# mmwillet/TTS.cpp

Hardware: AMD Instinct MI355X
Metric: audio-seconds/sec (Parler-TTS-Mini fp16, greedy decode + DAC to 44.1 kHz PCM) (higher is better)
Workload: dtype f16

## Files before the change

### tts.cpp_amd/csrc/dac_b3_kernels.h

```cpp
#pragma once
#include <hip/hip_runtime.h>
#include <stdint.h>
#include <type_traits>

struct ResUnitGeom { int C, KS, KS2, WST, n7, ns1, n1; };
__host__ __device__ inline ResUnitGeom resunit_geom(int C, int KS, int KS2) {
    ResUnitGeom g;
    g.C = C; g.KS = KS; g.KS2 = KS2;
    const int a = 3 * KS * 2 * C * 8, b = 3 * KS2 * 2 * 96 * 8;
    g.WST = a > b ? a : b;
    g.n7 = (C / 8) * (4 / KS);
    g.ns1 = (C / 16) / KS2;
    g.n1 = (C / 96) * g.ns1;
    return g;
}

static __global__ void pack_resunit_b3_kernel(const float *w7, const float *w1, __bf16 *dst, int C, int KS, int KS2) {
    const ResUnitGeom g = resunit_geom(C, KS, KS2);
    const int64_t per7 = (int64_t) KS * 2 * C * 8, per1 = (int64_t) KS2 * 2 * 96 * 8;
    const int64_t total = (int64_t) g.n7 * per7 + (int64_t) g.n1 * per1;
    for (int64_t i = (int64_t) blockIdx.x * blockDim.x + threadIdx.x; i < total; i += (int64_t) gridDim.x * blockDim.x) {
        float v = 0.0f;
        int64_t base, plane_sz;
        if (i < (int64_t) g.n7 * per7) {
// ... 30 lines not shown
        dst[base + 2 * plane_sz] = h3;
    }
}

template <int N, typename F>
__device__ __forceinline__ void static_for(F &&f) {
    if constexpr (N > 0) {
        static_for<N - 1>(f);
        f(std::integral_constant<int, N - 1>{});
    }
}

struct ResUnitArgs {
    const float *x;
    float *y;
    const __bf16 *w;
    const float *b7, *b1;
    const float *alpha_in;
    const float *alpha_mid;
    int L, dil, pad;
    const uint32_t *frames;
    int mult;
    long long *stamps;
};
#define RU_STAMP(k) do { if (a.stamps && tid == 0) a.stamps[((int64_t) blockIdx.z * gridDim.x + blockIdx.x) * 5 + (k)] = (long long) __builtin_readcyclecounter(); } while (0)

template <int MI, int KS, int KS2, int SCHED = 1, int ABL = 0>
__global__ __launch_bounds__(512, 2) void resunit_b3_kernel(ResUnitArgs a) {
    constexpr int C = 32 * MI, WN = 8, NT = 512, T_T = 32 * WN;
    constexpr int SPC = 4 / KS;
    constexpr int WPL7 = KS * 2 * C * 8, WPL1 = KS2 * 2 * 96 * 8;
    constexpr int WST = 3 * (WPL7 > WPL1 ? WPL7 : WPL1);
    constexpr int NCH = C / 8, N7 = NCH * SPC, NP = MI / 3, NS1 = (C / 16) / KS2, N1 = NP * NS1;
    constexpr int WV = (WST / 8 + NT - 1) / NT;
    static_assert(4 % KS == 0 && (C / 16) % KS2 == 0 && MI % 3 == 0, "stage shapes");
    extern __shared__ __attribute__((aligned(16))) char smem[];
    const int xw = T_T + 6 * a.dil;
    const int xpl = xw * 8;
    __bf16 *wsb = (__bf16 *) smem;
    __bf16 *xsb = wsb + 2 * WST;
    float4 *tab = (float4 *) (xsb + 2 * 3 * xpl);
    float2 *tin = (float2 *) (tab + C);
    const int tid = threadIdx.x, lane = tid & 63, wn = tid >> 6;
    const int l31 = lane & 31, hi = lane >> 5;
    const int t0 = blockIdx.x * T_T;
    const int LS = a.L, L = valid_len(a.frames, a.mult, a.L);
// ... 499 lines not shown
        }
}

static __global__ void pack_convt_w_b3_kernel(const float *src, __bf16 *dst, int cout, int cin, int S, int CO_T, int n_chunks, int scheme = 0) {
    const int64_t plane_sz = (int64_t) 2 * S * 2 * CO_T * 8;
    const int64_t total = (int64_t) ((cout + CO_T - 1) / CO_T) * n_chunks * plane_sz;
    for (int64_t i = (int64_t) blockIdx.x * blockDim.x + threadIdx.x; i < total; i += (int64_t) gridDim.x * blockDim.x) {
        const int j = (int) (i % 8);
        int64_t r = i / 8;
        const int col = (int) (r % CO_T); r /= CO_T;
        const int hi = (int) (r % 2); r /= 2;
        const int ph = (int) (r % S); r /= S;
        const int ks = (int) (r % 2); r /= 2;
        const int ch = (int) (r % n_chunks);
        const int ct = (int) (r / n_chunks);
        const int co = ct * CO_T + col, ci = ch * 16 + ks * 8 + j, k = ph + hi * S;
        float v = 0.0f;
        if (co < cout && ci < cin) v = src[((int64_t) ci * cout + co) * 2 * S + k];
        const int64_t base = ((int64_t) ct * n_chunks + ch) * split_planes(scheme) * plane_sz + (i % plane_sz);
        split_store(scheme, v, dst, base, plane_sz);
    }
}

template <int S, int MI, bool PLANES = false, typename SP = SplitB3>
__global__ __launch_bounds__(512, 2) void convt_b3_kernel(ConvTArgs a) {
    constexpr int NPL = SP::NPL;
    constexpr int CO_T = 32 * MI, WN = 8, TI_T = 32 * WN, NT = 64 * WN, K2 = 2 * S;
    constexpr int WPL = 2 * S * 2 * CO_T * 8;
    constexpr int WV = (NPL * WPL / 8 + NT - 1) / NT;
    constexpr int xw = TI_T + 1;
    constexpr int XR = (2 * xw + NT - 1) / NT;
    constexpr int xpl = 2 * xw * 8;
    extern __shared__ __attribute__((aligned(16))) char smem[];
    __bf16 *wsb = (__bf16 *) smem;
    __bf16 *xsb = wsb + 2 * NPL * WPL;
    float2 *tin = (float2 *) (xsb + 2 * NPL * xpl);
    const int tid = threadIdx.x, lane = tid & 63, wn = tid >> 6;
    const int l31 = lane & 31, hi = lane >> 5;
    const TileId tile = xcd_tile(a.npos, a.nco, a.nz);
    if (!tile.valid) return;
    const int ti0 = tile.pos * TI_T, co0 = tile.co * CO_T;
    const int n_chunks = a.cin / 16;
    const int LS = a.L, L = valid_len_z(a.frames, a.mult, a.L, tile.z);
    const int LoS = a.Lout, Lout = a.frames ? (L - 1) * S - 2 * a.pad + K2 : a.Lout;
    if (ti0 > L) return;
    const float *xg = a.x + (int64_t) tile.z * a.cin * LS;
    const int64_t psti = (int64_t) (a.cin / 8) * LS * 8;
    const __bf16 *xpg = PLANES ? a.xp + (int64_t) tile.z * NPL * psti : nullptr;
    float *yg = a.y + (int64_t) tile.z * a.cout * LoS;
    const uint4d *wg = (const uint4d *) ((const __bf16 *) a.w + (int64_t) tile.co * n_chunks * NPL * WPL);

    if (!PLANES) {
        for (int i = tid; i < a.cin; i += NT) {
            const float al = a.alpha ? a.alpha[i] : 1.0f;
            tin[i] = make_float2(al, 1.0f / al);
        }
    }

    float16d acc[MI][S];
#pragma unroll
    for (int i = 0; i < MI; i++)
#pragma unroll
        for (int ph = 0; ph < S; ph++)
#pragma unroll
            for (int e = 0; e < 16; e++) acc[i][ph][e] = 0.0f;

    uint4d wreg[WV];
    float xreg[PLANES ? 1 : XR][8];
    uint4d xpreg[PLANES ? XR : 1][NPL];
    auto prefetch = [&](int c) __attribute__((always_inline)) {
        const uint4d *wp = wg + (int64_t) c * (NPL * WPL / 8);
#pragma unroll
        for (int j = 0; j < WV; j++) {
            const int i = tid + j * NT;
            if (i < NPL * WPL / 8) wreg[j] = wp[i];
        }
#pragma unroll
        for (int q = 0; q < XR; q++) {
            const int u = tid + q * NT;
            const int g = u / xw, r = u - g * xw;
            const int ti = ti0 - 1 + r;
            const bool ok = g < 2 && ti >= 0 && ti < L;
            if constexpr (PLANES) {
                const uint4d zero = {0u, 0u, 0u, 0u};
#pragma unroll
                for (int pl = 0; pl < NPL; pl++)
                    xpreg[q][pl] = ok ? *(const uint4d *) (xpg + pl * psti + ((int64_t) (c * 2 + g) * LS + ti) * 8) : zero;
            } else {
#pragma unroll
                for (int e = 0; e < 8; e++) xreg[q][e] = ok ? xg[(int64_t) (c * 16 + g * 8 + e) * LS + ti] : 0.0f;
            }
        }
    };
    auto commit = [&](int c, int buf) __attribute__((always_inline)) {
        uint4d *wd = (uint4d *) (wsb + buf * NPL * WPL);
#pragma unroll
        for (int j = 0; j < WV; j++) {
            const int i = tid + j * NT;
            if (i < NPL * WPL / 8) wd[i] = wreg[j];
        }
        __bf16 *xd = xsb + buf * NPL * xpl;
#pragma unroll
        for (int q = 0; q < XR; q++) {
            const int u = tid + q * NT;
            const int g = u / xw, r = u - g * xw;
            if constexpr (PLANES) {
                if (g < 2) {
                    __bf16 *p = xd + (g * xw + r) * 8;
#pragma unroll
                    for (int pl = 0; pl < NPL; pl++) *(uint4d *) (p + pl * xpl) = xpreg[q][pl];
                }
            } else if (g < 2) {
                if (a.alpha) {
                    float al[8], ral[8];
#pragma unroll
                    for (int e = 0; e < 8; e++) { const float2 t2 = tin[c * 16 + g * 8 + e]; al[e] = t2.x; ral[e] = t2.y; }
                    snake_vec<8>(xreg[q], al, ral);
                }
                bf16x8d hp[NPL];
#pragma unroll
                for (int e = 0; e < 8; e++) {
                    __bf16 pv[NPL];
// ... 113 lines not shown
            if (s >= cnt) continue;
            v = w7[((int64_t) co * C + chunk * 16 + hi * 8 + j) * 7 + first + s];
            plane_sz = (int64_t) cnt * 2 * C * 8;
            base = (int64_t) st * WST + ((int64_t) (s * 2 + hi) * C + co) * 8 + j;
        } else {
            const int64_t i1 = i - (int64_t) n7 * slot7;
            const int st = (int) (i1 / per1);
            int64_t r = i1 % per1;
            const int m = (int) (r % 8); r /= 8;
            const int col = (int) (r % 96); r /= 96;
            const int hi = (int) (r % 2); r /= 2;
            const int s = (int) r;
            const int pass = st / ns1, q = st % ns1;
            const int ks = q * KS2 + s, ib = ks / 2, qq = ks % 2;
            const int ch = 32 * ib + 16 * qq + (m < 4 ? 4 * hi + m : 8 + 4 * hi + m - 4);
            v = w1[(int64_t) (96 * pass + col) * C + ch];
            plane_sz = per1;
            base = (int64_t) (n7 + st) * WST + (i1 % per1);
        }
        split_store(scheme, v, dst, base, plane_sz);
    }
}

__device__ __forceinline__ void dac_wait_vmcnt0() { asm volatile("s_waitcnt vmcnt(0)" ::: "memory"); }
template <int MI, int KS2, typename SP = SplitB3, bool WDMA = false, int VAR = 0, int NI = 1>
__global__ __launch_bounds__(512, 2) void resunit_t7_kernel(ResUnitArgs a) {
    constexpr int NPL = SP::NPL;
    using G = ResT7<MI>;
    constexpr int C = 32 * MI, WN = 8, NT = 512, T_T = 32 * WN * NI, NQ = NI + 1;
    constexpr int SPC = G::SPC, NCH = C / 16, N7 = NCH * SPC;
    constexpr int WPL1 = KS2 * 2 * 96 * 8;
    constexpr int WST = NPL * G::MAXCNT * 2 * C * 8;
    constexpr int NP = MI / 3, NS1 = (C / 16) / KS2, N1 = NP * NS1;
    constexpr int WV = (WST / 8 + NT - 1) / NT;
    static_assert(NPL * WPL1 <= WST && (C / 16) % KS2 == 0 && MI % 3 == 0, "stage shapes");
    static_assert(NI == 1 || ((VAR & 2) != 0 && NPL <= 2 && N1 % 2 == 0), "NI > 1: once-built operand, an even number of k = 1 stages");
    extern __shared__ __attribute__((aligned(16))) char smem[];
    const int xw = T_T + 6 * a.dil;
    const int xpl = 2 * xw * 8;
    __bf16 *wsb = (__bf16 *) smem;
    __bf16 *xsb = wsb + 2 * WST;
    float4 *tab = (float4 *) (xsb + 2 * NPL * xpl);
    float2 *tin = (float2 *) (tab + C);
    const int tid = threadIdx.x, lane = tid & 63, wn = tid >> 6;
    const int l31 = lane & 31, hi = lane >> 5;
    const int t0 = blockIdx.x * T_T;
    const int LS = a.L, L = valid_len(a.frames, a.mult, a.L);
    if (t0 >= L) return;
    const float *xg = a.x + (int64_t) blockIdx.z * C * LS;
    float *yg = a.y + (int64_t) blockIdx.z * C * LS;
    const uint4d *wg = (const uint4d *) a.w;

    for (int i = tid; i < C; i += NT) {
        const float am = a.alpha_mid[i], ai = a.alpha_in[i];
        tab[i] = make_float4(a.b7[i], am, 1.0f / am, a.b1[i]);
        tin[i] = make_float2(ai, 1.0f / ai);
    }

    float16d acc[NI][MI];
#pragma unroll
    for (int j = 0; j < NI; j++)
#pragma unroll
        for (int i = 0; i < MI; i++)
#pragma unroll
            for (int e = 0; e < 16; e++) acc[j][i][e] = 0.0f;

    constexpr int NPIECE = WST * 2 / 1024;
    static_assert(!WDMA || (WST * 2) % 1024 == 0, "stage = whole 1-KiB pieces");
    uint4d wreg[WDMA ? 1 : WV];
    float xreg[NQ][8];
    auto prefetch_w = [&](int g) __attribute__((always_inline)) {
        if constexpr (WDMA) {
            const char *wp = (const char *) a.w + (int64_t) g * (WST * 2) + lane * 16;
            char *wd = (char *) (wsb + (g & 1) * WST);
#pragma unroll
            for (int j = 0; j < (NPIECE + 7) / 8; j++) {
                const int pc = wn + 8 * j;
                if (NPIECE % 8 == 0 || pc < NPIECE)
                    __builtin_amdgcn_global_load_lds((const __attribute__((address_space(1))) void *) (wp + pc * 1024),
// ... 184 lines not shown
#pragma unroll
                for (int pl = 0; pl < NPL; pl++)
                    af[ii][pl] = *(const bf16x8d *) (ws + pl * WPL1 + (((s * 2 + hi) * 96) + ii * 32 + l31) * 8);
#pragma unroll
            for (int tm = 0; tm < SP::NT; tm++)
#pragma unroll
                for (int ii = 0; ii < 3; ii++)
                    acc2[ii] = SP::mfma(af[ii][SP::ta(tm)], bf[SP::tb(tm)], acc2[ii]);
        });
        if constexpr (g2 + 1 < N1 || jt + 1 < NI) {
            commit_w((N7 + g2 + 1) & 1);
            __syncthreads();
        }
        if constexpr (q == NS1 - 1) {
            if (t < L) {
#pragma unroll
                for (int i = 0; i < 3; i++) {
                    float rv[16];
#pragma unroll
                    for (int e = 0; e < 16; e++) {
                        const int co = 96 * p + 32 * i + (e & 3) + 8 * (e >> 2) + 4 * hi;
                        rv[e] = xg[(int64_t) co * LS + t];
                    }
#pragma unroll
                    for (int e = 0; e < 16; e++) {
                        const int co = 96 * p + 32 * i + (e & 3) + 8 * (e >> 2) + 4 * hi;
                        yg[(int64_t) co * LS + t] = (acc2[i][e] + tab[co].w) + rv[e];
                    }
                }
            }
        }
    });
    });
    RU_STAMP(4);
}
```

### tts.cpp_amd/csrc/dac_kernels.h

```cpp
#pragma once
#include <hip/hip_runtime.h>
#include <stdint.h>

typedef float float4d __attribute__((ext_vector_type(4)));

__device__ __forceinline__ float snake_sin_poly(float x) {
    const float q = rintf(x * 0.318309886183790671537767526745028724f);
    float r = fmaf(q, -3.140625f, x);
    r = fmaf(q, -0.0009670257568359375f, r);
    r = fmaf(q, -6.2771141529083251953e-07f, r);
    r = fmaf(q, -1.2154201256553420762e-10f, r);
    const float s = r * r;
    if (((int) q) & 1) r = -r;
    float u = 2.6083159809786593541503e-06f;
    u = fmaf(u, s, -0.0001981069071916863322258f);
    u = fmaf(u, s, 0.00833307858556509017944336f);
    u = fmaf(u, s, -0.166666597127914428710938f);
    return fmaf(s, u * r, r);
}
__device__ __forceinline__ float snake_sin(float x) {
    if (!(fabsf(x) < 125.0f)) return sinf(x);
    return snake_sin_poly(x);
}

__device__ __forceinline__ float snake_f(float x, float alpha, float ralpha) {
    const float s = snake_sin(x * alpha);
    return x + (s * s) * ralpha;
}
template <int N>
__device__ __forceinline__ void snake_vec(float (&v)[N], const float (&al)[N], const float (&ral)[N]) {
    float arg[N];
    bool big = false;
#pragma unroll
    for (int e = 0; e < N; e++) { arg[e] = v[e] * al[e]; big = big || !(fabsf(arg[e]) < 125.0f); }
    if (__builtin_amdgcn_ballot_w64(big) != 0) {
#pragma unroll
        for (int e = 0; e < N; e++) { const float s = snake_sin(arg[e]); v[e] = v[e] + (s * s) * ral[e]; }
    } else {
#pragma unroll
        for (int e = 0; e < N; e++) { const float s = snake_sin_poly(arg[e]); v[e] = v[e] + (s * s) * ral[e]; }
    }
}
__device__ __forceinline__ float snake_ch(float x, int cig, int cin, int cin_pad, const float *als, const float *alpha, int tab) {
    if (tab) return snake_f(x, als[cig], als[cin_pad + cig]);
    const float al = cig < cin ? alpha[cig] : 1.0f;
    return snake_f(x, al, 1.0f / al);
}

struct DacEmbedArgs {
    const uint32_t *frames;
    const uint32_t *codes;
    const float *codebook;
    const float *proj_w;
    const float *proj_b;
    int n_cb, cb_size, cb_dim, latent, T;
    int Tout;
    float *out;
    int x_f16;
};

static __global__ void dac_embed_kernel(DacEmbedArgs a) {
    const int t = blockIdx.x * blockDim.x + threadIdx.x;
    const int c = blockIdx.y, z = blockIdx.z;
// ... 1382 lines not shown
```

### tts.cpp_amd/csrc/shim_codec.hip

```cpp
#include "shim_internal.h"

#include "dac_kernels.h"
#include "dac_b3_kernels.h"
#include "kokoro_kernels.h"

static int dac_snapshot(tts_hip_ctx *c, int stage, const float *dev, size_t C, size_t L, size_t LS) {
    if (!c->debug) return 0;
    HIPCHK(hipStreamSynchronize(c->stream));
    std::vector<float> &v = c->dac_dbg[stage];
    v.resize(C * L);
    HIPCHK(hipMemcpy2DAsync(v.data(), L * 4, dev, LS * 4, L * 4, C, hipMemcpyDeviceToHost, c->stream));
    HIPCHK(hipStreamSynchronize(c->stream));
    return 0;
}

#define CI32_K1 16
#ifndef CI32_T
#define CI32_T 8
#endif
#ifndef CI32_K7
#define CI32_K7 4
#endif
static int conv_tile(int cout, int K, int *CO_T, int *CI_T) {
    if (K != 7 && K != 1) return -1;
// ... 327 lines not shown
        else if (K == 1) hipLaunchKernelGGL(conv1d_kernel<1>, grid, dim3(256), lds, c->stream, a);
        else return set_err("conv1d: kernel size %d unsupported", K);
        HIPCHK(hipGetLastError());
    }
    return prof_end(c);
}

template <int S, int MI, int WM, int WN, int CI_T>
static int launch_convt_mfma(tts_hip_ctx *c, const ConvTArgs &a_in, int nz) {
    constexpr int CO_T = 32 * MI * WM, TI_T = 32 * WN, WCH = CI_T * 2 * S * CO_T;
    const int cin_pad = (a_in.cin + CI_T - 1) / CI_T * CI_T;
    ConvTArgs a = a_in;
    const size_t lds = dac_lds_request(c, ((size_t) 2 * WCH + 2 * (size_t) ((CI_T * (TI_T + 1) + 3) & ~3)) * 4, (a.alpha ? 2 * (size_t) cin_pad : 0) * 4, &a.alpha_tab, true);
    static std::atomic<uint64_t> attr{0};
    if (attr_needed(attr, c->device)) {
        HIPCHK(hipFuncSetAttribute((const void *) convt1d_mfma_kernel<S, MI, WM, WN, CI_T>, hipFuncAttributeMaxDynamicSharedMemorySize, 160 * 1024));
    }
    const dim3 grid((a.L + 1 + TI_T - 1) / TI_T, (a.cout + CO_T - 1) / CO_T, nz);
    hipLaunchKernelGGL((convt1d_mfma_kernel<S, MI, WM, WN, CI_T>), grid, dim3(64 * WM * WN), lds, c->stream, a);
    HIPCHK(hipGetLastError());
    return 0;
}

template <int S, int MI, bool PL, typename SP>
static int launch_convt_b3_t(tts_hip_ctx *c, const ConvTArgs &a, int nz) {
    constexpr int CO_T = 32 * MI, WPL = 2 * S * 2 * CO_T * 8, xpl = 2 * 257 * 8;
    const size_t lds = (size_t) 2 * SP::NPL * WPL * 2 + (size_t) 2 * SP::NPL * xpl * 2 + (size_t) a.cin * 8;
    if (lds > 160 * 1024) return set_err("convt_b3: %d input channels need %zu bytes of LDS", a.cin, lds);
    static std::atomic<uint64_t> attr{0};
    if (attr_needed(attr, c->device)) {
        HIPCHK(hipFuncSetAttribute((const void *) convt_b3_kernel<S, MI, PL, SP>, hipFuncAttributeMaxDynamicSharedMemorySize, 160 * 1024));
    }
    ConvTArgs b = a;
    b.npos = (a.L + 1 + 255) / 256; b.nz = nz;
    b.nco = xcd_order(a.cout / CO_T, (double) a.cin * a.L * nz * 4, (double) a.cout * a.cin * 2 * S * 6);
    hipLaunchKernelGGL((convt_b3_kernel<S, MI, PL, SP>), dim3(xcd_grid(b.npos, a.cout / CO_T, b.nz)), dim3(512), lds, c->stream, b);
    HIPCHK(hipGetLastError());
    return 0;
}
template <int S, int MI, typename SP>
static int launch_convt_b3_s(tts_hip_ctx *c, const ConvTArgs &a, int nz) {
    return a.xp ? launch_convt_b3_t<S, MI, true, SP>(c, a, nz) : launch_convt_b3_t<S, MI, false, SP>(c, a, nz);
}
template <int S, int MI>
static int launch_convt_b3(tts_hip_ctx *c, const ConvTArgs &a, int nz) {
    const int sc = dac_scheme(c);
    return sc == 0 ? launch_convt_b3_s<S, MI, SplitB3>(c, a, nz) : sc == 1 ? launch_convt_b3_s<S, MI, SplitH2>(c, a, nz) : launch_convt_b3_s<S, MI, SplitH1>(c, a, nz);
}

static int launch_convt(tts_hip_ctx *c, ConvTArgs ta, size_t w_off, int nz) {
    const bool valu = (c->d.flags & TTS_HIP_FLAG_VALU_GEMM) != 0;
    const int s = ta.stride;
    auto pct = c->packed_ct.find(w_off);
    if (!valu && c->dac_convt_b3 && pct != c->packed_ct.end()) {
        ta.w = (const float *) pct->second;
        ta.x_f16 = 0;
        if (s == 8) return launch_convt_b3<8, 1>(c, ta, nz);
        if (s == 4) return launch_convt_b3<4, 2>(c, ta, nz);
        return launch_convt_b3<2, 3>(c, ta, nz);
    }
    int CO_T = 0;
    const int cfg = valu ? -1 : convt_tile(ta.cout, s, &CO_T);
    ta.x_f16 = c->dac_f16 ? 1 : 0;
    auto pk16 = c->packed16.find(w_off);
// ... 69 lines not shown
        else CHK((launch_conv_b3p_t<7, 2, 2, 1, 4, 4, 2>(c, a, bt.n)));
    } else if (cout % 256 == 0) {
        CHK((launch_conv_b3p_t<1, 4, 2, 2, 4, 1, 2>(c, a, bt.n)));
    } else {
        CHK((launch_conv_b3p_t<1, 2, 4, 2, 4, 1, 2>(c, a, bt.n)));
    }
    return prof_end(c);
}

template <int MI, int KS, int KS2>
static int launch_resunit_t(tts_hip_ctx *c, const ResUnitArgs &a, int nz) {
    constexpr int C = 32 * MI;
    const ResUnitGeom g = resunit_geom(C, KS, KS2);
    const int xw = 256 + 6 * a.dil;
    const size_t lds = (size_t) 2 * g.WST * 2 + (size_t) 6 * xw * 8 * 2 + (size_t) C * 24;
    static std::atomic<uint64_t> attr{0};
    if (attr_needed(attr, c->device)) {
        HIPCHK(hipFuncSetAttribute((const void *) resunit_b3_kernel<MI, KS, KS2>, hipFuncAttributeMaxDynamicSharedMemorySize, 160 * 1024));
    }
    hipLaunchKernelGGL((resunit_b3_kernel<MI, KS, KS2>), dim3((a.L + 255) / 256, 1, nz), dim3(512), lds, c->stream, a);
    HIPCHK(hipGetLastError());
    return 0;
}
template <int MI, int KS2, typename SP, bool WDMA, int VAR, int NI = 1>
static int launch_resunit_t7_s(tts_hip_ctx *c, const ResUnitArgs &a, int nz) {
    constexpr int C = 32 * MI, T_T = 256 * NI;
    const int xw = T_T + 6 * a.dil;
    const size_t WST = (size_t) SP::NPL * ResT7<MI>::MAXCNT * 2 * C * 8;
    const size_t lds = 2 * WST * 2 + (size_t) 2 * SP::NPL * 2 * xw * 8 * 2 + (size_t) C * 24;
    static std::atomic<uint64_t> attr{0};
    if (attr_needed(attr, c->device)) {
        HIPCHK(hipFuncSetAttribute((const void *) resunit_t7_kernel<MI, KS2, SP, WDMA, VAR, NI>, hipFuncAttributeMaxDynamicSharedMemorySize, 160 * 1024));
    }
    hipLaunchKernelGGL((resunit_t7_kernel<MI, KS2, SP, WDMA, VAR, NI>), dim3((a.L + T_T - 1) / T_T, 1, nz), dim3(512), lds, c->stream, a);
    HIPCHK(hipGetLastError());
    return 0;
}
template <int MI, int KS2>
static int launch_resunit_t7(tts_hip_ctx *c, const ResUnitArgs &a, int nz) {
    const int sc = dac_scheme(c);
    constexpr int NI = MI == 3 ? 2 : 1;
    if (c->dac_wdma)
        return sc == 0 ? launch_resunit_t7_s<MI, KS2, SplitB3, true, 0>(c, a, nz) : sc == 1 ? launch_resunit_t7_s<MI, KS2, SplitH2, true, 2, NI>(c, a, nz) : launch_resunit_t7_s<MI, KS2, SplitH1, true, 2, NI>(c, a, nz);
    return sc == 0 ? launch_resunit_t7_s<MI, KS2, SplitB3, false, 0>(c, a, nz) : sc == 1 ? launch_resunit_t7_s<MI, KS2, SplitH2, false, 0>(c, a, nz) : launch_resunit_t7_s<MI, KS2, SplitH1, false, 0>(c, a, nz);
}
static bool resunit_fused(const tts_hip_ctx *c, const DRes &r, int dil) {
    return c->dac_fuse && !(c->d.flags & TTS_HIP_FLAG_VALU_GEMM) && dil <= 9 && c->packed_ru.count(r.in_w);
}
static int launch_resunit(tts_hip_ctx *c, const DacBatch &bt, const DRes &r, int C, int LS, int dil, const float *x, float *y) {
    ResUnitArgs a{};
    a.x = x; a.y = y; a.w = c->packed_ru.at(r.in_w);
    a.b7 = (const float *) (c->arena + r.in_b); a.b1 = (const float *) (c->arena + r.out_b);
    a.alpha_in = (const float *) (c->arena + r.in_alpha); a.alpha_mid = (const float *) (c->arena + r.out_alpha);
    a.L = LS; a.dil = dil; a.pad = 3 * dil; a.frames = bt.frames; a.mult = bt.mult;
    const double Lv = bt.tot_frames * bt.mult;
    CHK(prof_begin(c, TTS_HIP_K_DAC_RESUNIT, (2.0 * C * Lv + 8.0 * C * C) * 4, 2.0 * C * (double) C * 8 * Lv));
    if (c->dac_tap7) {
        if (C == 96) CHK((launch_resunit_t7<3, 3>(c, a, bt.n)));
        else CHK((launch_resunit_t7<6, 4>(c, a, bt.n)));
    } else if (C == 96) CHK((launch_resunit_t<3, 4, 3>(c, a, bt.n)));
    else CHK((launch_resunit_t<6, 2, 4>(c, a, bt.n)));
    return prof_end(c);
}

static int dac_decode_batch_on(tts_hip_ctx *c, const uint32_t *codes, const uint32_t *frames, uint32_t n, float *pcm_out);
static int dac_decode_batch(tts_hip_ctx *c, const uint32_t *codes, const uint32_t *frames, uint32_t n, float *pcm_out) {
    if (!c || !c->finalized || !c->has_dac) return set_err("tts_hip_dac_decode: context has no finalized DAC");
    if (!frames || !codes || !pcm_out) return set_err("tts_hip_dac_decode: null argument");
    const uint32_t G = (uint32_t) std::max(1, c->dac_group);
    size_t code_off = 0, pcm_off = 0;
    for (uint32_t g0 = 0; g0 < n; g0 += G) {
        const uint32_t m = std::min(G, n - g0);
        size_t fr = 0;
        for (uint32_t i = 0; i < m; i++) fr += frames[g0 + i];
        int rc;
        {
            std::lock_guard<std::mutex> lock(g_dac_pass_mutex[(unsigned) c->device % 64]);
            if (!c->dac_stream) {
                rc = dac_decode_batch_on(c, codes + code_off * c->d_ncb, frames + g0, m, pcm_out + pcm_off);
// ... 111 lines not shown
    if (c->packed_p.count(c->d_initw) && !(c->d.flags & TTS_HIP_FLAG_VALU_GEMM)) {
        CHK(launch_split(c, bt, cur, c->d_latent, LS, 0, false, (__bf16 *) t2));
        const bool pl = convt_takes_planes(0);
        CHK(launch_conv_planes(c, bt, (const __bf16 *) t2, c->d_latent, LS, c->d_initw, c->d_initb, c->d_c0, 7, 1, nullptr, (!pl || (c->debug && n == 1)) ? t1 : nullptr,
                               pl ? (__bf16 *) B.dplanes : nullptr, pl ? c->dblocks[0].alpha : 0, pl));
        if (pl) convt_in = (const __bf16 *) B.dplanes;
    } else
    CHK(launch_conv(c, bt, cur, c->d_latent, LS, c->d_initw, c->d_initb, 0, false, c->d_c0, 7, 3, 1, nullptr, false, t1));
    std::swap(cur, t1);
    if (n == 1) CHK(dac_snapshot(c, 1, cur, (size_t) c->d_c0, (size_t) L, (size_t) LS));

    int C = c->d_c0;
    for (size_t bi = 0; bi < c->dblocks.size(); bi++) {
        const DBlock &b = c->dblocks[bi];
        const int Lout = (L - 1) * b.stride - 2 * b.padding + 2 * b.stride, LSout = dac_row_stride(c, Lout);
        ConvTArgs ta{};
        ta.x = cur; ta.w = (const float *) (c->arena + b.w); ta.b = (const float *) (c->arena + b.b);
        ta.alpha = (const float *) (c->arena + b.alpha); ta.y = t1; ta.cin = b.cin; ta.cout = b.cout; ta.L = LS;
        ta.Lout = LSout; ta.stride = b.stride; ta.pad = b.padding;
        ta.frames = c->d_frames; ta.mult = bt.mult;
        ta.xp = convt_in;
        convt_in = nullptr;
        const double Lov = bt.tot_frames * bt.mult * b.stride;
        CHK(prof_begin(c, TTS_HIP_K_DAC_CONVT, ((double) b.cin * bt.tot_frames * bt.mult + (double) b.cout * Lov + (double) b.cin * b.cout * 2 * b.stride) * 4,
                       2.0 * b.cin * (double) b.cout * 2 * Lov));
        CHK(launch_convt(c, ta, b.w, (int) n));
        CHK(prof_end(c));
        std::swap(cur, t1);
        L = Lout; LS = LSout; C = b.cout;
        bt.mult *= b.stride;
        if (c->packed_p.count(b.res[0].in_w) && !(c->d.flags & TTS_HIP_FLAG_VALU_GEMM)) {
            __bf16 *PA = (__bf16 *) t2, *PB = (__bf16 *) B.dplanes;
            CHK(launch_split(c, bt, cur, C, LS, b.res[0].in_alpha, true, PA));
            for (int r = 0; r < 3; r++) {
                int dil = 1;
                for (int e = 0; e < r; e++) dil *= 3;
                CHK(launch_conv_planes(c, bt, PA, C, LS, b.res[r].in_w, b.res[r].in_b, C, 7, dil, nullptr, nullptr, PB, b.res[r].out_alpha, true));
                const bool to_convt = r == 2 && convt_takes_planes(bi + 1);
                const bool want_y = r < 2 || !to_convt || (c->debug && n == 1);
                CHK(launch_conv_planes(c, bt, PB, C, LS, b.res[r].out_w, b.res[r].out_b, C, 1, 1, cur, want_y ? t1 : nullptr, (r < 2 || to_convt) ? PA : nullptr,
                                       r < 2 ? b.res[r + 1].in_alpha : (to_convt ? c->dblocks[bi + 1].alpha : 0), r < 2 || to_convt));
                if (to_convt) convt_in = PA;
                if (want_y) std::swap(cur, t1);
            }
            if (n == 1) CHK(dac_snapshot(c, 2 + (int) bi, cur, (size_t) C, (size_t) L, (size_t) LS));
            continue;
        }
        for (int r = 0; r < 3; r++) {
            int dil = 1;
            for (int e = 0; e < r; e++) dil *= 3;
            if (resunit_fused(c, b.res[r], dil)) {
                CHK(launch_resunit(c, bt, b.res[r], C, LS, dil, cur, t1));
                std::swap(cur, t1);
                continue;
            }
            CHK(launch_conv(c, bt, cur, C, LS, b.res[r].in_w, b.res[r].in_b, b.res[r].in_alpha, true, C, 7, 3 * dil, dil, nullptr, false, t1,
                            b.res[r].out_alpha, true));
            CHK(launch_conv(c, bt, t1, C, LS, b.res[r].out_w, b.res[r].out_b, 0, false, C, 1, 0, 1, cur, false, t2));
            std::swap(cur, t2);
        }
        if (n == 1) CHK(dac_snapshot(c, 2 + (int) bi, cur, (size_t) C, (size_t) L, (size_t) LS));
    }
    CHK(launch_conv(c, bt, cur, C, LS, c->d_fw, c->d_fb, c->d_falpha, true, 1, 7, 3, 1, nullptr, true, t1));
    HIPCHK(hipMemcpyAsync(B.h_pcm, t1, (size_t) n * LS * 4, hipMemcpyDeviceToHost, c->stream));
    HIPCHK(hipStreamSynchronize(c->stream));
    size_t off = 0;
    for (uint32_t i = 0; i < n; i++) {
        memcpy(pcm_out + off, B.h_pcm + (size_t) i * LS, (size_t) frames[i] * c->d_up * 4);
        off += (size_t) frames[i] * c->d_up;
    }
    return 0;
}

extern "C" int tts_hip_dac_decode(tts_hip_ctx *c, const uint32_t *codes, uint32_t frames, float *pcm_out) {
    return dac_decode_batch(c, codes, &frames, 1, pcm_out);
}
// ... 851 lines not shown
```

### tts.cpp_amd/csrc/shim_core.hip

```cpp
#include "shim_internal.h"

static thread_local char g_err[1024] = "";
int set_err(const char *fmt, ...) {
    va_list ap;
    va_start(ap, fmt);
    vsnprintf(g_err, sizeof(g_err), fmt, ap);
    va_end(ap);
    return -1;
}

extern "C" const char *tts_hip_last_error(void) { return g_err; }
extern "C" const char *tts_hip_version(void) { return "tts_hip 0.1 (gfx950)"; }

static float h2f_host(uint16_t h) {
    const uint32_t sign = (uint32_t) (h & 0x8000u) << 16;
    uint32_t exp = (h >> 10) & 0x1F, man = h & 0x3FF, bits;
    if (exp == 0) {
        if (man == 0) bits = sign;
        else {
            exp = 113;
            while ((man & 0x400) == 0) { man <<= 1; exp--; }
            bits = sign | (exp << 23) | ((man & 0x3FF) << 13);
        }
    } else if (exp == 31) bits = sign | 0x7F800000u | (man << 13);
// ... 94 lines not shown
    if (const char *e = getenv("TTS_HIP_DAC_BF16X3")) (void) tts_hip_tune(c, "dac_exact_fp32", atoi(e) == 0);
    if (const char *e = getenv("TTS_HIP_DAC_SPLIT")) c->dac_split = atoi(e) != 0;
    if (const char *e = getenv("TTS_HIP_GEN_COMPACT")) c->gen_compact = atoi(e) != 0;
    if (const char *e = getenv("TTS_HIP_TILE_FORCE")) c->tile_force = atoi(e);
    if (const char *e = getenv("TTS_HIP_TILE_KS")) c->tile_force_ks = atoi(e);
    if (const char *e = getenv("TTS_HIP_GEMV_ROWS")) c->gemv_rows = atoi(e) != 0;
    if (const char *e = getenv("TTS_HIP_LLAMA_GRAPH")) c->llama_graph = atoi(e) != 0;
    if (const char *e = getenv("TTS_HIP_Q4_NATIVE")) c->q4_native = atoi(e) != 0;
    return c;
}

extern "C" int tts_hip_tune(tts_hip_ctx *c, const char *key, int v) {
    if (!c || !key) return set_err("tts_hip_tune: null argument");
    const std::string k(key);
    if (k == "dac_exact_fp32") {
        c->dac_b3 = v ? 0 : 2; c->dac_fuse = c->dac_convt_b3 = c->dac_planes = v ? 0 : 1;
    } else if (k == "dac_fuse") c->dac_fuse = v;
    else if (k == "dac_convt_b3") c->dac_convt_b3 = v;
    else if (k == "dac_convt_planes") c->dac_convt_planes = v;
    else if (k == "dac_planes") c->dac_planes = v;
    else if (k == "dac_split") c->dac_split = v ? 1 : 0;
    else if (k == "dac_f16_planes") c->dac_f16_planes = v;
    else if (k == "dac_tap7") c->dac_tap7 = v;
    else if (k == "dac_wdma") c->dac_wdma = v;
    else if (k == "dac_b3") c->dac_b3 = std::max(0, v);
    else if (k == "dac_conv1_direct") c->dac_conv1_direct = v != 0;
    else if (k == "kokoro_mfma") c->kk_mfma = v != 0;
    else if (k == "kokoro_b3") c->kk_b3 = v != 0;
    else if (k == "kokoro_attn_lds") c->kk_attn_lds = v != 0;
    else if (k == "kokoro_split") {
        if (c->kk_split != (v != 0)) { (void) hipDeviceSynchronize(); for (auto &pw : c->packed_b3) free_dev(pw.second); c->packed_b3.clear(); }
        c->kk_split = v != 0;
    }
    else if (k == "kokoro_lstm_split") c->kk_lstm_split = v != 0;
    else if (k == "kokoro_adain_split") c->kk_adain_split = v != 0;
    else if (k == "ln_fuse_max") c->ln_fuse_max = std::max(0, std::min(32, v));
    else if (k == "attn_short") c->attn_short = v != 0;
    else if (k == "attn_rows_min") c->attn_rows_min = std::max(0, v);
    else if (k == "attn_fused") c->attn_fused = v != 0;
    else if (k == "attn_split") c->attn_split_max = std::max(1, std::min(16, v));
    else if (k == "attn_fold") c->attn_fold = v != 0;
    else if (k == "attn_wave") c->attn_wave = v != 0;
    else if (k == "cross_fold") c->cross_fold = v != 0;
    else if (k == "tile_min_rows") c->tile_min_rows = std::max(0, v);
    else if (k == "tile_deep") c->tile_deep = v;
    else if (k == "qtile_min_rows") c->qtile_min_rows = std::max(0, v);
// ... 751 lines not shown
```

### tts.cpp_amd/csrc/shim_internal.h

```cpp
#pragma once
#include "../../include/tts_hip.h"

#include <hip/hip_runtime.h>

#include <algorithm>
#include <atomic>
#include <cmath>
#include <cstdarg>
#include <cstdio>
#include <cstdlib>
#include <cstring>
#include <map>
#include <set>
#include <mutex>
#include <string>
#include <vector>

#include <unordered_map>
#define LLAMA_GREEDY_CHUNK 8

int set_err(const char *fmt, ...);
#define HIPCHK(expr)                                                                          \
    do {                                                                                      \
        hipError_t _e = (expr);                                                               \
// ... 37 lines not shown
};

struct DRes { size_t in_alpha, in_w, in_b, out_alpha, out_w, out_b; };
struct DBlock { int stride, padding, cin, cout; size_t alpha, w, b; DRes res[3]; };

struct CopyItem { size_t dst; std::string src; size_t src_off = 0; size_t bytes = 0; };

struct ProfEv { hipEvent_t a, b; int kclass; };

constexpr int GRAPH_KEY_ROWS = 8192;

struct DacBuffers {
    float *dbuf[3] = {nullptr, nullptr, nullptr};
    size_t dbuf_elems = 0;
    size_t cap_codes = 0;
    float *dplanes = nullptr;
    uint32_t *d_codes = nullptr;
    float *h_pcm = nullptr;
    size_t h_pcm_elems = 0;
    int users = 0;
};
extern DacBuffers g_dac_buffers[64];
extern std::mutex g_dac_pass_mutex[64];

struct tts_hip_ctx {
    int device = 0;
    hipStream_t stream = nullptr;
    hipStream_t dac_stream = nullptr;
    tts_hip_desc d{};
    std::map<std::string, Tensor> tensors;
    bool planned = false, finalized = false, weights_present = false;
    bool has_parler = false, has_dac = false;

    char *arena = nullptr;
    size_t arena_bytes = 0;
    bool arena_external = false;
    bool arena_counted = false;
    std::vector<CopyItem> copies;

    int H = 0, L = 0, NH = 0, F = 0, V = 0, NO = 0, NCTX = 0, E = 0, ECAP = 0, PV = 0, EROWS = 0, NPOS = 0, KVPOS = 0;
    W embed_prompts, embed_tokens, heads;
    size_t pos_embed = 0, text_enc = 0, ln_w = 0, ln_b = 0, cross_kv = 0;
    char *cond_text_enc = nullptr, *cond_cross_kv = nullptr;
    char *text_enc_ptr() const { return cond_text_enc ? cond_text_enc : arena + text_enc; }
    char *cross_kv_ptr() const { return cond_cross_kv ? cond_cross_kv : arena + cross_kv; }
    std::vector<PLayer> layers;
// ... 176 lines not shown
    uint32_t *d_tokens_out = nullptr;
    size_t tokens_out_cap = 0;
    uint8_t *d_eos = nullptr;
    uint32_t *h_ids = nullptr, *h_pos = nullptr, *h_seq = nullptr, *h_tok = nullptr;
    float *h_logits = nullptr;
    std::vector<uint32_t> host_pos;

    size_t dac_frame_elems = 0;
    size_t dac_cap_frames = 0;
    uint32_t *d_frames = nullptr;
    size_t d_frames_cap = 0;
    bool debug = false;
    std::map<int, std::vector<float>> dac_dbg;
    std::vector<float> win_pcm;
    std::map<size_t, float *> packed;
    std::set<size_t> packed_direct;
    std::map<size_t, _Float16 *> packed16;
    std::map<size_t, __bf16 *> packed_b3;
    std::map<size_t, __bf16 *> packed_ru;
    std::map<size_t, __bf16 *> packed_p;
    int dac_split = 1;
    int dac_f16_planes = 1;
    int dac_tap7 = 1;
    int dac_wdma = 1;
    int dac_planes = 1;
    bool dac_buf_user = false;
    std::map<size_t, __bf16 *> packed_ct;
    int dac_convt_planes = 1;
    int dac_convt_b3 = 1;
    int dac_fuse = 1;
    int dac_b3 = 2;
    bool kk_lstm_split = true;
    char *kk_pool = nullptr;
    size_t kk_pool_cap = 0, kk_pool_next = 0;
    int *kk_stuck = nullptr;
    bool kk_b3 = true;
    bool kk_attn_lds = true;
    int kk_split = 1;
    bool kk_adain_split = true;
    bool kk_mfma = true;
    bool attn_short = true;
    int dac_group = 64;
    bool dac_conv1_direct = true;
    int attn_rows_min = 256;
    int tile_min_rows = 33;
    int tile_force = -1;
// ... 77 lines not shown
```

Baseline: 1025.

## Emit snake-split bf16 planes from last resunit and DMA convT weights into LDS

The last residual unit of a 192-channel DAC block now applies the next block's snake activation and writes the split bf16 plane layout the following transposed conv consumes, so the fp32 output write, re-read and separate plane conversion can be skipped. The transposed-conv kernel gains a path that loads weights straight into LDS with global_load_lds instead of staging them through registers. The snake sine-squared polynomial is also folded into a single helper. Both paths are on by default through a new dac_lean bitmask, and they add template variants and more LDS per block.

```diff
diff --git a/tts.cpp_amd/csrc/dac_b3_kernels.h b/tts.cpp_amd/csrc/dac_b3_kernels.h
--- a/tts.cpp_amd/csrc/dac_b3_kernels.h
+++ b/tts.cpp_amd/csrc/dac_b3_kernels.h
@@ -76,6 +76,8 @@
     const uint32_t *frames;
     int mult;
     long long *stamps;
+    __bf16 *yp;
+    const float *alpha_out;
 };
 #define RU_STAMP(k) do { if (a.stamps && tid == 0) a.stamps[((int64_t) blockIdx.z * gridDim.x + blockIdx.x) * 5 + (k)] = (long long) __builtin_readcyclecounter(); } while (0)
 
@@ -621,7 +623,8 @@
     }
 }
 
-template <int S, int MI, bool PLANES = false, typename SP = SplitB3>
+__device__ __forceinline__ void dac_wait_vmcnt0() { asm volatile("s_waitcnt vmcnt(0)" ::: "memory"); }
+template <int S, int MI, bool PLANES = false, typename SP = SplitB3, bool WDMA = false>
 __global__ __launch_bounds__(512, 2) void convt_b3_kernel(ConvTArgs a) {
     constexpr int NPL = SP::NPL;
     constexpr int CO_T = 32 * MI, WN = 8, TI_T = 32 * WN, NT = 64 * WN, K2 = 2 * S;
@@ -664,15 +667,29 @@
 #pragma unroll
             for (int e = 0; e < 16; e++) acc[i][ph][e] = 0.0f;
 
-    uint4d wreg[WV];
+    constexpr int NPIECE = NPL * WPL * 2 / 1024;
+    static_assert((NPL * WPL * 2) % 1024 == 0, "stage = whole 1-KiB pieces");
+    uint4d wreg[WDMA ? 1 : WV];
     float xreg[PLANES ? 1 : XR][8];
     uint4d xpreg[PLANES ? XR : 1][NPL];
     auto prefetch = [&](int c) __attribute__((always_inline)) {
-        const uint4d *wp = wg + (int64_t) c * (NPL * WPL / 8);
-#pragma unroll
-        for (int j = 0; j < WV; j++) {
-            const int i = tid + j * NT;
-            if (i < NPL * WPL / 8) wreg[j] = wp[i];
+        if constexpr (WDMA) {
+            const char *wp = (const char *) (wg + (int64_t) c * (NPL * WPL / 8)) + lane * 16;
+            char *wd = (char *) (wsb + (c & 1) * NPL * WPL);
+#pragma unroll
+            for (int j = 0; j < (NPIECE + 7) / 8; j++) {
+                const int pc = wn + 8 * j;
+                if (NPIECE % 8 == 0 || pc < NPIECE)
+                    __builtin_amdgcn_global_load_lds((const __attribute__((address_space(1))) void *) (wp + pc * 1024),
+                                                     (__attribute__((address_space(3))) void *) (wd + pc * 1024), 16, 0, 0);
+            }
+        } else {
+            const uint4d *wp = wg + (int64_t) c * (NPL * WPL / 8);
+#pragma unroll
+            for (int j = 0; j < WV; j++) {
+                const int i = tid + j * NT;
+                if (i < NPL * WPL / 8) wreg[j] = wp[i];
+            }
         }
 #pragma unroll
         for (int q = 0; q < XR; q++) {
@@ -692,11 +709,15 @@
         }
     };
     auto commit = [&](int c, int buf) __attribute__((always_inline)) {
-        uint4d *wd = (uint4d *) (wsb + buf * NPL * WPL);
-#pragma unroll
-        for (int j = 0; j < WV; j++) {
-            const int i = tid + j * NT;
-            if (i < NPL * WPL / 8) wd[i] = wreg[j];
+        if constexpr (WDMA) {
+            dac_wait_vmcnt0();
+        } else {
+            uint4d *wd = (uint4d *) (wsb + buf * NPL * WPL);
+#pragma unroll
+            for (int j = 0; j < WV; j++) {
+                const int i = tid + j * NT;
+                if (i < NPL * WPL / 8) wd[i] = wreg[j];
+            }
         }
         __bf16 *xd = xsb + buf * NPL * xpl;
 #pragma unroll
@@ -856,8 +877,7 @@
     }
 }
 
-__device__ __forceinline__ void dac_wait_vmcnt0() { asm volatile("s_waitcnt vmcnt(0)" ::: "memory"); }
-template <int MI, int KS2, typename SP = SplitB3, bool WDMA = false, int VAR = 0, int NI = 1>
+template <int MI, int KS2, typename SP = SplitB3, bool WDMA = false, int VAR = 0, int NI = 1, bool YPL = false>
 __global__ __launch_bounds__(512, 2) void resunit_t7_kernel(ResUnitArgs a) {
     constexpr int NPL = SP::NPL;
     using G = ResT7<MI>;
@@ -876,19 +896,21 @@
     __bf16 *xsb = wsb + 2 * WST;
     float4 *tab = (float4 *) (xsb + 2 * NPL * xpl);
     float2 *tin = (float2 *) (tab + C);
+    float2 *tout = tin + C;
     const int tid = threadIdx.x, lane = tid & 63, wn = tid >> 6;
     const int l31 = lane & 31, hi = lane >> 5;
     const int t0 = blockIdx.x * T_T;
     const int LS = a.L, L = valid_len(a.frames, a.mult, a.L);
     if (t0 >= L) return;
     const float *xg = a.x + (int64_t) blockIdx.z * C * LS;
-    float *yg = a.y + (int64_t) blockIdx.z * C * LS;
+    float *yg = YPL && !a.y ? nullptr : a.y + (int64_t) blockIdx.z * C * LS;
     const uint4d *wg = (const uint4d *) a.w;
 
     for (int i = tid; i < C; i += NT) {
         const float am = a.alpha_mid[i], ai = a.alpha_in[i];
         tab[i] = make_float4(a.b7[i], am, 1.0f / am, a.b1[i]);
         tin[i] = make_float2(ai, 1.0f / ai);
+        if constexpr (YPL) { const float ao = a.alpha_out[i]; tout[i] = make_float2(ao, 1.0f / ao); }
     }
 
     float16d acc[NI][MI];
@@ -1119,11 +1141,44 @@
                         const int co = 96 * p + 32 * i + (e & 3) + 8 * (e >> 2) + 4 * hi;
                         rv[e] = xg[(int64_t) co * LS + t];
                     }
+                    if constexpr (YPL) {
+                        typedef __bf16 bf16x4d __attribute__((ext_vector_type(4)));
+                        const int64_t psto = (int64_t) (C / 8) * LS * 8;
+                        __bf16 *ypz = a.yp + (int64_t) blockIdx.z * NPL * psto;
+#pragma unroll
+                        for (int qd = 0; qd < 4; qd++) {
+                            const int cq = 96 * p + 32 * i + 8 * qd + 4 * hi;
+                            float v[4], al[4], ral[4];
+#pragma unroll
+                            for (int r = 0; r < 4; r++) {
+                                v[r] = (acc2[i][4 * qd + r] + tab[cq + r].w) + rv[4 * qd + r];
+                                const float2 to = tout[cq + r];
+                                al[r] = to.x; ral[r] = to.y;
+                            }
+                            if (a.y) {
+#pragma unroll
+                                for (int r = 0; r < 4; r++) yg[(int64_t) (cq + r) * LS + t] = v[r];
+                            }
+                            snake_vec<4>(v, al, ral);
+                            bf16x4d hp[NPL];
+#pragma unroll
+                            for (int r = 0; r < 4; r++) {
+                                __bf16 pv[NPL];
+                                SP::split(v[r], pv);
+#pragma unroll
+                                for (int pl = 0; pl < NPL; pl++) hp[pl][r] = pv[pl];
+                            }
+                            __bf16 *pp = ypz + ((int64_t) (cq >> 3) * LS + t) * 8 + (cq & 7);
+#pragma unroll
+                            for (int pl = 0; pl < NPL; pl++) *(bf16x4d *) (pp + pl * psto) = hp[pl];
+                        }
+                    } else {
 #pragma unroll
                     for (int e = 0; e < 16; e++) {
                         const int co = 96 * p + 32 * i + (e & 3) + 8 * (e >> 2) + 4 * hi;
                         yg[(int64_t) co * LS + t] = (acc2[i][e] + tab[co].w) + rv[e];
                     }
+                    }
                 }
             }
         }
diff --git a/tts.cpp_amd/csrc/dac_kernels.h b/tts.cpp_amd/csrc/dac_kernels.h
--- a/tts.cpp_amd/csrc/dac_kernels.h
+++ b/tts.cpp_amd/csrc/dac_kernels.h
@@ -22,10 +22,27 @@
     if (!(fabsf(x) < 125.0f)) return sinf(x);
     return snake_sin_poly(x);
 }
+__device__ __forceinline__ float snake_sin2_poly(float x) {
+    const float q = rintf(x * 0.318309886183790671537767526745028724f);
+    float r = fmaf(q, -3.140625f, x);
+    r = fmaf(q, -0.0009670257568359375f, r);
+    r = fmaf(q, -6.2771141529083251953e-07f, r);
+    r = fmaf(q, -1.2154201256553420762e-10f, r);
+    const float s = r * r;
+    float u = 2.6083159809786593541503e-06f;
+    u = fmaf(u, s, -0.0001981069071916863322258f);
+    u = fmaf(u, s, 0.00833307858556509017944336f);
+    u = fmaf(u, s, -0.166666597127914428710938f);
+    const float p = fmaf(s, u * r, r);
+    return p * p;
+}
+__device__ __forceinline__ float snake_sin2(float x) {
+    if (!(fabsf(x) < 125.0f)) { const float s = sinf(x); return s * s; }
+    return snake_sin2_poly(x);
+}
 
 __device__ __forceinline__ float snake_f(float x, float alpha, float ralpha) {
-    const float s = snake_sin(x * alpha);
-    return x + (s * s) * ralpha;
+    return x + snake_sin2(x * alpha) * ralpha;
 }
 template <int N>
 __device__ __forceinline__ void snake_vec(float (&v)[N], const float (&al)[N], const float (&ral)[N]) {
@@ -35,10 +52,10 @@
     for (int e = 0; e < N; e++) { arg[e] = v[e] * al[e]; big = big || !(fabsf(arg[e]) < 125.0f); }
     if (__builtin_amdgcn_ballot_w64(big) != 0) {
 #pragma unroll
-        for (int e = 0; e < N; e++) { const float s = snake_sin(arg[e]); v[e] = v[e] + (s * s) * ral[e]; }
+        for (int e = 0; e < N; e++) v[e] = v[e] + snake_sin2(arg[e]) * ral[e];
     } else {
 #pragma unroll
-        for (int e = 0; e < N; e++) { const float s = snake_sin_poly(arg[e]); v[e] = v[e] + (s * s) * ral[e]; }
+        for (int e = 0; e < N; e++) v[e] = v[e] + snake_sin2_poly(arg[e]) * ral[e];
     }
 }
 __device__ __forceinline__ float snake_ch(float x, int cig, int cin, int cin_pad, const float *als, const float *alpha, int tab) {
diff --git a/tts.cpp_amd/csrc/shim_codec.hip b/tts.cpp_amd/csrc/shim_codec.hip
--- a/tts.cpp_amd/csrc/shim_codec.hip
+++ b/tts.cpp_amd/csrc/shim_codec.hip
@@ -373,24 +373,25 @@
     return 0;
 }
 
-template <int S, int MI, bool PL, typename SP>
+template <int S, int MI, bool PL, typename SP, bool WDMA = false>
 static int launch_convt_b3_t(tts_hip_ctx *c, const ConvTArgs &a, int nz) {
     constexpr int CO_T = 32 * MI, WPL = 2 * S * 2 * CO_T * 8, xpl = 2 * 257 * 8;
     const size_t lds = (size_t) 2 * SP::NPL * WPL * 2 + (size_t) 2 * SP::NPL * xpl * 2 + (size_t) a.cin * 8;
     if (lds > 160 * 1024) return set_err("convt_b3: %d input channels need %zu bytes of LDS", a.cin, lds);
     static std::atomic<uint64_t> attr{0};
     if (attr_needed(attr, c->device)) {
-        HIPCHK(hipFuncSetAttribute((const void *) convt_b3_kernel<S, MI, PL, SP>, hipFuncAttributeMaxDynamicSharedMemorySize, 160 * 1024));
+        HIPCHK(hipFuncSetAttribute((const void *) convt_b3_kernel<S, MI, PL, SP, WDMA>, hipFuncAttributeMaxDynamicSharedMemorySize, 160 * 1024));
     }
     ConvTArgs b = a;
     b.npos = (a.L + 1 + 255) / 256; b.nz = nz;
     b.nco = xcd_order(a.cout / CO_T, (double) a.cin * a.L * nz * 4, (double) a.cout * a.cin * 2 * S * 6);
-    hipLaunchKernelGGL((convt_b3_kernel<S, MI, PL, SP>), dim3(xcd_grid(b.npos, a.cout / CO_T, b.nz)), dim3(512), lds, c->stream, b);
+    hipLaunchKernelGGL((convt_b3_kernel<S, MI, PL, SP, WDMA>), dim3(xcd_grid(b.npos, a.cout / CO_T, b.nz)), dim3(512), lds, c->stream, b);
     HIPCHK(hipGetLastError());
     return 0;
 }
 template <int S, int MI, typename SP>
 static int launch_convt_b3_s(tts_hip_ctx *c, const ConvTArgs &a, int nz) {
+    if (a.xp && (c->dac_lean & DAC_LEAN_CONVT_WDMA)) return launch_convt_b3_t<S, MI, true, SP, true>(c, a, nz);
     return a.xp ? launch_convt_b3_t<S, MI, true, SP>(c, a, nz) : launch_convt_b3_t<S, MI, false, SP>(c, a, nz);
 }
 template <int S, int MI>
@@ -506,17 +507,17 @@
     HIPCHK(hipGetLastError());
     return 0;
 }
-template <int MI, int KS2, typename SP, bool WDMA, int VAR, int NI = 1>
+template <int MI, int KS2, typename SP, bool WDMA, int VAR, int NI = 1, bool YPL = false>
 static int launch_resunit_t7_s(tts_hip_ctx *c, const ResUnitArgs &a, int nz) {
     constexpr int C = 32 * MI, T_T = 256 * NI;
     const int xw = T_T + 6 * a.dil;
     const size_t WST = (size_t) SP::NPL * ResT7<MI>::MAXCNT * 2 * C * 8;
-    const size_t lds = 2 * WST * 2 + (size_t) 2 * SP::NPL * 2 * xw * 8 * 2 + (size_t) C * 24;
+    const size_t lds = 2 * WST * 2 + (size_t) 2 * SP::NPL * 2 * xw * 8 * 2 + (size_t) C * (YPL ? 32 : 24);
     static std::atomic<uint64_t> attr{0};
     if (attr_needed(attr, c->device)) {
-        HIPCHK(hipFuncSetAttribute((const void *) resunit_t7_kernel<MI, KS2, SP, WDMA, VAR, NI>, hipFuncAttributeMaxDynamicSharedMemorySize, 160 * 1024));
-    }
-    hipLaunchKernelGGL((resunit_t7_kernel<MI, KS2, SP, WDMA, VAR, NI>), dim3((a.L + T_T - 1) / T_T, 1, nz), dim3(512), lds, c->stream, a);
+        HIPCHK(hipFuncSetAttribute((const void *) resunit_t7_kernel<MI, KS2, SP, WDMA, VAR, NI, YPL>, hipFuncAttributeMaxDynamicSharedMemorySize, 160 * 1024));
+    }
+    hipLaunchKernelGGL((resunit_t7_kernel<MI, KS2, SP, WDMA, VAR, NI, YPL>), dim3((a.L + T_T - 1) / T_T, 1, nz), dim3(512), lds, c->stream, a);
     HIPCHK(hipGetLastError());
     return 0;
 }
@@ -524,6 +525,9 @@
 static int launch_resunit_t7(tts_hip_ctx *c, const ResUnitArgs &a, int nz) {
     const int sc = dac_scheme(c);
     constexpr int NI = MI == 3 ? 2 : 1;
+    if constexpr (MI == 6) {
+        if (a.yp) return sc == 1 ? launch_resunit_t7_s<MI, KS2, SplitH2, true, 2, NI, true>(c, a, nz) : launch_resunit_t7_s<MI, KS2, SplitH1, true, 2, NI, true>(c, a, nz);
+    }
     if (c->dac_wdma)
         return sc == 0 ? launch_resunit_t7_s<MI, KS2, SplitB3, true, 0>(c, a, nz) : sc == 1 ? launch_resunit_t7_s<MI, KS2, SplitH2, true, 2, NI>(c, a, nz) : launch_resunit_t7_s<MI, KS2, SplitH1, true, 2, NI>(c, a, nz);
     return sc == 0 ? launch_resunit_t7_s<MI, KS2, SplitB3, false, 0>(c, a, nz) : sc == 1 ? launch_resunit_t7_s<MI, KS2, SplitH2, false, 0>(c, a, nz) : launch_resunit_t7_s<MI, KS2, SplitH1, false, 0>(c, a, nz);
@@ -531,14 +535,19 @@
 static bool resunit_fused(const tts_hip_ctx *c, const DRes &r, int dil) {
     return c->dac_fuse && !(c->d.flags & TTS_HIP_FLAG_VALU_GEMM) && dil <= 9 && c->packed_ru.count(r.in_w);
 }
-static int launch_resunit(tts_hip_ctx *c, const DacBatch &bt, const DRes &r, int C, int LS, int dil, const float *x, float *y) {
+static bool resunit_planes_out(const tts_hip_ctx *c, int C) {
+    return (c->dac_lean & DAC_LEAN_RU_PLANES) && C == 192 && c->dac_tap7 && c->dac_wdma && dac_scheme(c) != 0;
+}
+static int launch_resunit(tts_hip_ctx *c, const DacBatch &bt, const DRes &r, int C, int LS, int dil, const float *x, float *y, __bf16 *yp = nullptr,
+                          size_t alpha_out = 0) {
     ResUnitArgs a{};
     a.x = x; a.y = y; a.w = c->packed_ru.at(r.in_w);
+    a.yp = yp; a.alpha_out = yp ? (const float *) (c->arena + alpha_out) : nullptr;
     a.b7 = (const float *) (c->arena + r.in_b); a.b1 = (const float *) (c->arena + r.out_b);
     a.alpha_in = (const float *) (c->arena + r.in_alpha); a.alpha_mid = (const float *) (c->arena + r.out_alpha);
     a.L = LS; a.dil = dil; a.pad = 3 * dil; a.frames = bt.frames; a.mult = bt.mult;
     const double Lv = bt.tot_frames * bt.mult;
-    CHK(prof_begin(c, TTS_HIP_K_DAC_RESUNIT, (2.0 * C * Lv + 8.0 * C * C) * 4, 2.0 * C * (double) C * 8 * Lv));
+    CHK(prof_begin(c, TTS_HIP_K_DAC_RESUNIT, ((double) C * Lv * (4 + (y ? 4 : 0) + (yp ? 2 * split_planes(dac_scheme(c)) : 0)) + 8.0 * C * C * 4), 2.0 * C * (double) C * 8 * Lv));
     if (c->dac_tap7) {
         if (C == 96) CHK((launch_resunit_t7<3, 3>(c, a, bt.n)));
         else CHK((launch_resunit_t7<6, 4>(c, a, bt.n)));
@@ -696,7 +705,8 @@
         ta.xp = convt_in;
         convt_in = nullptr;
         const double Lov = bt.tot_frames * bt.mult * b.stride;
-        CHK(prof_begin(c, TTS_HIP_K_DAC_CONVT, ((double) b.cin * bt.tot_frames * bt.mult + (double) b.cout * Lov + (double) b.cin * b.cout * 2 * b.stride) * 4,
+        const double in_bytes = ta.xp ? 2.0 * split_planes(dac_scheme(c)) : 4.0;
+        CHK(prof_begin(c, TTS_HIP_K_DAC_CONVT, (double) b.cin * bt.tot_frames * bt.mult * in_bytes + ((double) b.cout * Lov + (double) b.cin * b.cout * 2 * b.stride) * 4,
                        2.0 * b.cin * (double) b.cout * 2 * Lov));
         CHK(launch_convt(c, ta, b.w, (int) n));
         CHK(prof_end(c));
@@ -724,8 +734,11 @@
             int dil = 1;
             for (int e = 0; e < r; e++) dil *= 3;
             if (resunit_fused(c, b.res[r], dil)) {
-                CHK(launch_resunit(c, bt, b.res[r], C, LS, dil, cur, t1));
-                std::swap(cur, t1);
+                const bool to_convt = r == 2 && resunit_planes_out(c, C) && convt_takes_planes(bi + 1);
+                const bool want_y = !to_convt || (c->debug && n == 1);
+                CHK(launch_resunit(c, bt, b.res[r], C, LS, dil, cur, want_y ? t1 : nullptr, to_convt ? (__bf16 *) t2 : nullptr, to_convt ? c->dblocks[bi + 1].alpha : 0));
+                if (to_convt) convt_in = (const __bf16 *) t2;
+                if (want_y) std::swap(cur, t1);
                 continue;
             }
             CHK(launch_conv(c, bt, cur, C, LS, b.res[r].in_w, b.res[r].in_b, b.res[r].in_alpha, true, C, 7, 3 * dil, dil, nullptr, false, t1,
diff --git a/tts.cpp_amd/csrc/shim_core.hip b/tts.cpp_amd/csrc/shim_core.hip
--- a/tts.cpp_amd/csrc/shim_core.hip
+++ b/tts.cpp_amd/csrc/shim_core.hip
@@ -140,6 +140,7 @@
     else if (k == "dac_split") c->dac_split = v ? 1 : 0;
     else if (k == "dac_f16_planes") c->dac_f16_planes = v;
     else if (k == "dac_tap7") c->dac_tap7 = v;
+    else if (k == "dac_lean") c->dac_lean = v == 1 ? DAC_LEAN_ALL : (v & DAC_LEAN_ALL);
     else if (k == "dac_wdma") c->dac_wdma = v;
     else if (k == "dac_b3") c->dac_b3 = std::max(0, v);
     else if (k == "dac_conv1_direct") c->dac_conv1_direct = v != 0;
diff --git a/tts.cpp_amd/csrc/shim_internal.h b/tts.cpp_amd/csrc/shim_internal.h
--- a/tts.cpp_amd/csrc/shim_internal.h
+++ b/tts.cpp_amd/csrc/shim_internal.h
@@ -83,6 +83,8 @@
 };
 extern DacBuffers g_dac_buffers[64];
 extern std::mutex g_dac_pass_mutex[64];
+
+enum { DAC_LEAN_RU_PLANES = 2, DAC_LEAN_CONVT_WDMA = 8, DAC_LEAN_ALL = DAC_LEAN_RU_PLANES | DAC_LEAN_CONVT_WDMA };
 
 struct tts_hip_ctx {
     int device = 0;
@@ -305,6 +307,7 @@
     int dac_split = 1;
     int dac_f16_planes = 1;
     int dac_tap7 = 1;
+    int dac_lean = DAC_LEAN_ALL;
     int dac_wdma = 1;
     int dac_planes = 1;
     bool dac_buf_user = false;
```

New measurement: 1035 (median of 6 runs). 1.0% higher.
